# twitter-research/cwn

Hardware: AMD Instinct MI355X
Metric: cells/sec, propagate scope, ZINC-like ring-lifted batch (max_ring 6) (higher is better)
Workload: dtype f32

## Files before the change

cwn_amd/csrc/cwn_layer.hip:

```cpp
#include <hip/hip_runtime.h>
#include <stdint.h>
#include <stddef.h>
#include <mutex>
#include <type_traits>
#include "../../include/cwn_hip.h"
#include "cwn_split.h"

namespace {

using cwn::frag_cd;

#ifdef CWN_LAYER_W8
#undef CWN_LAYER_THREADS
#define CWN_LAYER_THREADS 512
#define CWN_W8 1
#else
#define CWN_W8 0
#endif
#ifndef CWN_LAYER_THREADS
#define CWN_LAYER_THREADS 1024
#endif
#ifndef CWN_LAYER_WEARLY
#define CWN_LAYER_WEARLY -1
#endif
#ifndef CWN_LAYER_NT_STORE
#define CWN_LAYER_NT_STORE 1
#endif
#ifndef CWN_LAYER_WBAR
#define CWN_LAYER_WBAR 1
#endif
constexpr int kThreads = CWN_LAYER_THREADS;
static_assert(kThreads == 512 || kThreads == 1024, "8 or 16 waves");
constexpr int kWaves = kThreads / 64;
constexpr bool kW8 = CWN_W8 != 0;
constexpr int kHS = kThreads == 1024 ? 2 : 1;
constexpr int kWSets = kW8 ? 1 : 2 / kHS;
constexpr size_t kLdsBudget = kW8 ? CWN_LAYER_W8_LDS_BYTES : 160 * 1024;
__host__ __device__ constexpr int gemm_rows_cap(int F) { return kW8 ? CWN_LAYER_W8_GEMM_ROWS(F) : CWN_LAYER_GEMM_ROWS(F); }
__host__ __device__ constexpr int source_rows_cap(int F) { return kW8 ? CWN_LAYER_W8_SOURCE_ROWS(F) : CWN_LAYER_SOURCE_ROWS(F); }
constexpr int kEcap = CWN_LAYER_MAX_ENTRIES;
constexpr int kEI = kEcap / kThreads;
constexpr int kTaskRows = CWN_LAYER_TASK_ROWS;

enum { I_FLAGS = 0, I_G, I_GR0, I_GN, I_CR0, I_CN, I_UE0, I_UNE, I_NT, I_TASK0, I_R1 = 23, I_ROWS, I_B1, I_B2, I_TOTAL };
enum { T_DIM = 0, T_R0, T_N, T_BE0, T_BNE, T_SR0, T_SN, T_INTS };

enum { S_XG = 0, S_XC, S_UP_INDEX, S_UP_SHARED, S_UP_E, S_WP, S_MSG_BIAS, S_PAD, S_TASK0 };
enum { ST_X = 0, ST_XS, ST_OUT_UP, ST_OUT_B, ST_B_INDEX, ST_B_E, ST_EPS1, ST_EPS2, ST_OUT_D, ST_EPS3, ST_FIELDS };
constexpr int kSetFields = S_TASK0 + 2 * ST_FIELDS;
constexpr int kMaxSets = CWN_LAYER_MAX_DIMS;

struct BigSet {
    const int32_t* up_rowptr; const int32_t* up_col; const int32_t* up_aux;
    const int32_t* b_rowptr[2]; const int32_t* b_col[2];
    float* y1; float* y2;
};

struct LayerArgs {
    uint64_t set[kMaxSets][kSetFields];
    const int32_t* items;
    int32_t* err;
    unsigned char* csr_cache;
    int32_t rows_cap;
    int32_t xrows_cap;
    int32_t set_start1, set_start2;
    int32_t lds_limit;
    int32_t store_y;
    BigSet big[kMaxSets];
#ifdef CWN_LAYER_TIMING
    unsigned long long* stamps;
#endif
};

#ifdef CWN_LAYER_TIMING
#define CWN_STAMP_REC 96
#define CWN_STAMP(k)                                                                   \
    do {                                                                               \
        if (threadIdx.x == 0 && A.stamps != nullptr)                                   \
            A.stamps[(size_t)blockIdx.x * CWN_STAMP_REC + (k)] = __builtin_amdgcn_s_memtime();    \
    } while (0)
#define CWN_WSTAMP(k)                                                                  \
    do {                                                                               \
        if ((threadIdx.x & 63) == 0 && A.stamps != nullptr)                            \
            A.stamps[(size_t)blockIdx.x * CWN_STAMP_REC + 16 + 16 * (k) + (threadIdx.x >> 6)] = __builtin_amdgcn_s_memtime(); \
    } while (0)
#define CWN_RSTAMP(k)                                                                  \
    do {                                                                               \
        if ((threadIdx.x & 63) == 0 && A.stamps != nullptr)                            \
            A.stamps[(size_t)blockIdx.x * CWN_STAMP_REC + 64 + 16 * (k) + (threadIdx.x >> 6)] = __builtin_amdgcn_s_memrealtime(); \
    } while (0)
#else
#define CWN_STAMP(k) do { } while (0)
#define CWN_WSTAMP(k) do { } while (0)
#define CWN_RSTAMP(k) do { } while (0)
#endif

template <int F> struct Geo {
    static constexpr int kPlaneStride = F + 8;
    static constexpr int kYStride = F + 4;
    static constexpr int kKS = F / 32;
    static constexpr int kNCT = F / 16;
    static constexpr int kWPC = kWaves / kNCT / kHS;
    static constexpr int kG = F / 4;
    static constexpr int kNG = kThreads / kG;
    static constexpr int kNX = gemm_rows_cap(F) / kNG;
    static constexpr int kNE = source_rows_cap(F) / kNG;
    static_assert(gemm_rows_cap(F) % kNG == 0 && source_rows_cap(F) % kNG == 0, "caps are whole rounds");
    static constexpr int kMaxT = kW8 ? CWN_LAYER_W8_HALF_ROWS(F) / 16 / kWPC : gemm_rows_cap(F) / 16 / kWPC;
    static constexpr int kWChunks = 2 * kKS * 3;
    __host__ __device__ static constexpr size_t planes_bytes(int rows) { return (size_t)3 * rows * kPlaneStride * 2; }
    __host__ __device__ static constexpr size_t xrows_bytes(int rows) { return (size_t)(rows + 1) * F * 4; }
};

constexpr int kRpStride = kTaskRows + 2;
constexpr size_t kCntBytes = ((size_t)3 * kRpStride * 4 + 15) & ~(size_t)15;
constexpr size_t kIdxBytes = kCntBytes + (size_t)3 * kEcap * 2 + (size_t)3 * kRpStride * 2;
constexpr int kCsrSlot = CWN_LAYER_CSR_SLOT_BYTES;
static_assert(kCsrSlot >= 2 * kEcap * 2 + 3 * kRpStride * 2 && kCsrSlot % 16 == 0, "slot holds scol, saux, rowptr");
enum { kSort = 0, kSortStore = 1, kLoad = 2 };

template <int F>
__host__ __device__ constexpr size_t lds_bytes(int rows, int xrows) {
    return Geo<F>::planes_bytes(rows) + Geo<F>::xrows_bytes(xrows) + ((kIdxBytes + 15) & ~(size_t)15);
}

typedef float v4f __attribute__((ext_vector_type(4)));
typedef uint32_t v4u __attribute__((ext_vector_type(4)));
typedef const __attribute__((address_space(1))) float* gcf_p;
typedef __attribute__((address_space(1))) float* gf_p;
typedef const __attribute__((address_space(1))) int64_t* gci64_p;
typedef const __attribute__((address_space(1))) v4f* gcv4_p;
typedef const __attribute__((address_space(1))) v4u* gcu4_p;
typedef __attribute__((address_space(1))) v4f* gv4_p;
typedef const __attribute__((address_space(1))) unsigned char* gcb_p;
typedef __attribute__((address_space(1))) unsigned char* gb_p;
typedef const __attribute__((address_space(1))) uint64_t* gcu64_p;
typedef __attribute__((address_space(1))) v4u* gu4_p;

__device__ __forceinline__ float4 ldg4(gcf_p p) {
    const v4f v = *(gcv4_p)p;
    return make_float4(v.x, v.y, v.z, v.w);
}
__device__ __forceinline__ uint4 ldgu4(gcb_p p) {
    const v4u v = *(gcu4_p)p;
    return make_uint4(v.x, v.y, v.z, v.w);
}
__device__ __forceinline__ void stg4(gf_p p, const float4& a) {
    const v4f v = {a.x, a.y, a.z, a.w};
    *(gv4_p)p = v;
}
__device__ __forceinline__ float4 ldg4o(gcb_p base, uint32_t off) {
    const v4f v = *(gcv4_p)(base + off);
    return make_float4(v.x, v.y, v.z, v.w);
}
__device__ __forceinline__ uint4 ldgu4o(gcb_p base, uint32_t off) {
    const v4u v = *(gcu4_p)(base + off);
    return make_uint4(v.x, v.y, v.z, v.w);
}
__device__ __forceinline__ void stg4o(gb_p base, uint32_t off, const float4& a) {
    const v4f v = {a.x, a.y, a.z, a.w};
#if CWN_LAYER_NT_STORE
    __builtin_nontemporal_store(v, (gv4_p)(base + off));
#else
    *(gv4_p)(base + off) = v;
#endif
}
__device__ __forceinline__ float4 lds4(const float* p) { return *reinterpret_cast<const float4*>(p); }
__device__ __forceinline__ float4 sel4(bool c, const float4& a, const float4& b) {
    return make_float4(c ? a.x : b.x, c ? a.y : b.y, c ? a.z : b.z, c ? a.w : b.w);
}
template <int NX>
__device__ __forceinline__ float4 pick(const float4 (&xv)[NX], int k) {
    float4 r = xv[0];
#pragma unroll
    for (int i = 1; i < NX; ++i) r = sel4(k == i, xv[i], r);
    return r;
}

template <int NR>
struct RowSet { int s[NR], e[NR]; bool on[NR]; };

template <int NR, int NG>
// ... 256 lines not shown
                    for (int i = 0; i < kPer; ++i) {
                        const int lr = gq + i * G::kNG;
                        uint2 ph, pm, pl;
                        cwn::split4(cur[i], ph, pm, pl);
                        uint16_t* dst = bplanes + (size_t)lr * G::kPlaneStride + f;
                        *reinterpret_cast<uint2*>(dst) = ph;
                        *reinterpret_cast<uint2*>(dst + bplane) = pm;
                        *reinterpret_cast<uint2*>(dst + 2 * bplane) = pl;
                    }
                    if (c0 + kCH < n_max) request(nxt, c0 + kCH);
                    __syncthreads();
#pragma unroll
                    for (int hh = 0; hh < kWSets; ++hh) {
                        const int h = kHS == 2 ? my_h : hh;
                        const int rows_h = h == 0 ? g_n : c_n;
                        float* const yb = h == 0 ? Bg.y1 + (size_t)t_r0[0] * F : Bg.y2 + (size_t)c_r0 * F;
                        for (int tl = rt_par; tl < kCH / 16; tl += G::kWPC) {
                            if (c0 + tl * 16 >= rows_h) break;
                            const uint16_t* p0 = bplanes + (size_t)(h * kCH + tl * 16 + l15) * G::kPlaneStride + kq * 8;
                            frag_cd c = {0.f, 0.f, 0.f, 0.f};
#pragma unroll
                            for (int ks = 0; ks < G::kKS; ++ks) {
                                const uint4 xh = *reinterpret_cast<const uint4*>(p0 + ks * 32);
                                const uint4 xm = *reinterpret_cast<const uint4*>(p0 + bplane + ks * 32);
                                const uint4 xl = *reinterpret_cast<const uint4*>(p0 + 2 * bplane + ks * 32);
                                c = cwn::mfma_split6(wsp[hh][ks][0], wsp[hh][ks][1], wsp[hh][ks][2], xh, xm, xl, c);
                            }
                            if (h == 0) { c[0] += bb.x; c[1] += bb.y; c[2] += bb.z; c[3] += bb.w; }
                            const int row = c0 + tl * 16 + l15;
                            if (row < rows_h)
                                *reinterpret_cast<float4*>(yb + (size_t)row * F + ct * 16 + kq * 4) = make_float4(c[0], c[1], c[2], c[3]);
                        }
                    }
#pragma unroll
                    for (int i = 0; i < kPer; ++i) cur[i] = nxt[i];
                }
            }
            __builtin_amdgcn_fence(__ATOMIC_RELEASE, "workgroup");
            __syncthreads();
            __builtin_amdgcn_fence(__ATOMIC_ACQUIRE, "workgroup");
            int32_t* const lidx = reinterpret_cast<int32_t*>(smem);
            const int lcap = A.lds_limit / 4;
            int lused = 0;
            struct Seg { const int32_t* rp; const int32_t* cl; const int32_t* ax; int off; };
            auto stage = [&](const int32_t* rp_g, const int32_t* cl_g, const int32_t* ax_g, int first, int n_rows) {
                if (rp_g == nullptr || n_rows <= 0) return Seg{nullptr, nullptr, nullptr, 0};
                Seg sg{rp_g + first, cl_g, ax_g, 0};
                const int s0 = rp_g[first], e0 = rp_g[first + n_rows], ne = e0 - s0;
                const int need = (n_rows + 1) + ne * (ax_g != nullptr ? 2 : 1);
#ifdef CWN_BIG_NO_STAGE
                if (true) return sg;
#endif
                if (ne < 0 || lused + need > lcap) return sg;
                int32_t* lrp = lidx + lused;
                int32_t* lcl = lrp + n_rows + 1;
                int32_t* lax = lcl + ne;
                for (int i = tid; i <= n_rows; i += kThreads) lrp[i] = rp_g[first + i];
                for (int i = tid; i < ne; i += kThreads) {
                    lcl[i] = cl_g[s0 + i];
                    if (ax_g != nullptr) lax[i] = ax_g[s0 + i];
                }
                lused += need;
                return Seg{lrp, lcl, ax_g != nullptr ? lax : nullptr, s0};
            };
            const Seg su = (has_gemm) ? stage(Bg.up_rowptr, Bg.up_col, Bg.up_aux, t_r0[0], g_n) : Seg{nullptr, nullptr, nullptr, 0};
            Seg sb[2];
#pragma unroll
            for (int t = 0; t < 2; ++t)
                sb[t] = t_bne[t] > 0 ? stage(Bg.b_rowptr[t], Bg.b_col[t], nullptr, t_r0[t], t_n[t]) : Seg{nullptr, nullptr, nullptr, 0};
            __syncthreads();
            bool bad_big = false;
#pragma unroll
            for (int t = 0; t < 2; ++t) {
                if (t_n[t] == 0) continue;
                const gcf_p e1p = (gcf_p)sfld(S_TASK0 + t * ST_FIELDS + ST_EPS1), e2p = (gcf_p)sfld(S_TASK0 + t * ST_FIELDS + ST_EPS2);
                const float eps1 = e1p != (gcf_p)0 ? *e1p : 0.f, eps2 = e2p != (gcf_p)0 ? *e2p : 0.f;
                const gcf_p e3p = (gcf_p)sfld(S_TASK0 + t * ST_FIELDS + ST_EPS3);
                const float eps3 = e3p != (gcf_p)0 ? *e3p : 0.f;
                const gb_p o_d = (gb_p)sfld(S_TASK0 + t * ST_FIELDS + ST_OUT_D);
                const gcb_p xt = (gcb_p)sfld(S_TASK0 + t * ST_FIELDS + ST_X), xs = (gcb_p)sfld(S_TASK0 + t * ST_FIELDS + ST_XS);
                const gb_p o_up = (gb_p)sfld(S_TASK0 + t * ST_FIELDS + ST_OUT_UP), o_b = (gb_p)sfld(S_TASK0 + t * ST_FIELDS + ST_OUT_B);
                const Seg B_ = sb[t];
                const bool upper = t == 0 && has_gemm && su.rp != nullptr;
                const int s_lo = fld(I_TASK0 + t * T_INTS + T_SR0), s_n = t_sn[t];
                for (int r = gq; r < t_n[t]; r += G::kNG) {
                    const int64_t row = (int64_t)t_r0[t] + r;
                    const float4 xi = ldg4o(xt, (uint32_t)row * kRowB + fB);
                    float4 ab = make_float4(0.f, 0.f, 0.f, 0.f);
                    if (B_.rp != nullptr) {
                        const int s_ = B_.rp[r], e_ = B_.rp[r + 1];
                        for (int p = s_; p < e_; p += 4) {
                            int v[4];
                            float4 a[4];
#pragma unroll
                            for (int u = 0; u < 4; ++u) {
                                v[u] = B_.cl[min(p + u, e_ - 1) - B_.off];
                                if ((unsigned)(v[u] - s_lo) >= (unsigned)s_n) { bad_big = true; v[u] = s_lo; }
                            }
#pragma unroll
                            for (int u = 0; u < 4; ++u) a[u] = ldg4o(xs, (uint32_t)v[u] * kRowB + fB);
#pragma unroll
                            for (int u = 0; u < 4; ++u)
                                if (p + u < e_) { ab.x += a[u].x; ab.y += a[u].y; ab.z += a[u].z; ab.w += a[u].w; }
                        }
                    }
                    stg4o(o_b, (uint32_t)row * kRowB + fB, axpy4(ab, 1.0f + eps2, xi));
                    if (o_d != (gb_p)0)
                        stg4o(o_d, (uint32_t)row * kRowB + fB, axpy4(make_float4(0.f, 0.f, 0.f, 0.f), 1.0f + eps3, xi));
                    float4 au = make_float4(0.f, 0.f, 0.f, 0.f);
                    if (upper) {
                        const int s_ = su.rp[r], e_ = su.rp[r + 1];
                        for (int p = s_; p < e_; p += 4) {
                            int j[4], ci[4];
                            float4 y[4], z[4];
#pragma unroll
                            for (int u = 0; u < 4; ++u) {
                                j[u] = su.cl[min(p + u, e_ - 1) - su.off];
                                ci[u] = su.ax[min(p + u, e_ - 1) - su.off];
                                if ((unsigned)(j[u] - t_r0[0]) >= (unsigned)g_n || (unsigned)(ci[u] - c_r0) >= (unsigned)c_n) {
                                    bad_big = true;
                                    j[u] = t_r0[0]; ci[u] = c_r0;
                                }
                            }
#pragma unroll
                            for (int u = 0; u < 4; ++u) {
                                y[u] = *reinterpret_cast<const float4*>(Bg.y1 + (size_t)j[u] * F + f);
                                z[u] = *reinterpret_cast<const float4*>(Bg.y2 + (size_t)ci[u] * F + f);
                            }
#pragma unroll
                            for (int u = 0; u < 4; ++u)
                                if (p + u < e_) {
                                    au.x += fmaxf(y[u].x + z[u].x, 0.0f); au.y += fmaxf(y[u].y + z[u].y, 0.0f);
                                    au.z += fmaxf(y[u].z + z[u].z, 0.0f); au.w += fmaxf(y[u].w + z[u].w, 0.0f);
                                }
                        }
                    }
                    stg4o(o_up, (uint32_t)row * kRowB + fB, axpy4(au, 1.0f + eps1, xi));
                }
            }
            if (bad_big) atomicOr(A.err, CWN_ERR_BIT_BLOCK);
            CWN_RSTAMP(1);
            return;
        }
    }
    const bool fits = kW8 ? ((unsigned)rows_pad <= (unsigned)gemm_rows_cap(F) && (unsigned)x_rows <= (unsigned)source_rows_cap(F) &&
                             lds_bytes<F>(rows_pad, x_rows) <= (size_t)A.lds_limit)
                          : ((unsigned)rows_pad <= (unsigned)rows_cap && (unsigned)x_rows <= (unsigned)xrows_cap);
    if (!fits || (unsigned)total > (unsigned)kEcap ||
        (unsigned)t_n[0] > (unsigned)kTaskRows || (unsigned)t_n[1] > (unsigned)kTaskRows || (unsigned)R1 > (unsigned)rows_pad) {
        if (tid == 0) atomicOr(A.err, CWN_ERR_BIT_BLOCK);
        return;
    }
    bool bad = false;
    if constexpr (MODE != kLoad) {
        for (int i = tid; i < 3 * kRpStride; i += kThreads) ecnt[i] = 0u;
    }

    const gcf_p dummy = (gcf_p)A.items;
    int64_t ek[kEI], ev[kEI], ea[kEI];
    int s1 = 0, s2 = 0, s3 = 0;
    if constexpr (MODE != kLoad) {
        const int u_e0 = fld(I_UE0), t_be0[2] = {fld(I_TASK0 + T_BE0), fld(I_TASK0 + T_INTS + T_BE0)};
        s1 = fld(I_UNE), s2 = b1 + t_bne[0], s3 = b2 + t_bne[1];
        const gci64_p up_index = (gci64_p)sfld(S_UP_INDEX), up_shared = (gci64_p)sfld(S_UP_SHARED);
        const gci64_p b_index0 = (gci64_p)sfld(S_TASK0 + ST_B_INDEX);
        const gci64_p b_index1 = (gci64_p)sfld(S_TASK0 + ST_FIELDS + ST_B_INDEX);
        const int64_t up_E = (int64_t)sfld(S_UP_E);
        const int64_t b_E0 = (int64_t)sfld(S_TASK0 + ST_B_E), b_E1 = (int64_t)sfld(S_TASK0 + ST_FIELDS + ST_B_E);
#pragma unroll
        for (int i = 0; i < kEI; ++i) {
            const int w = tid + i * kThreads;
            const bool in_up = w < s1, in_b0 = w >= b1 && w < s2, in_b1 = w >= b2 && w < s3;
            const gci64_p src = in_up ? up_index : in_b0 ? b_index0 : in_b1 ? b_index1 : (gci64_p)A.items;
            const int64_t E = in_up ? up_E : in_b0 ? b_E0 : in_b1 ? b_E1 : 0;
            const int64_t e = in_up ? (int64_t)u_e0 + w : in_b0 ? (int64_t)t_be0[0] + (w - b1)
                                                       : in_b1 ? (int64_t)t_be0[1] + (w - b2) : 0;
            ev[i] = src[e];
            ek[i] = src[E + e];
            ea[i] = (in_up ? up_shared : (gci64_p)A.items)[in_up ? e : 0];
        }
    }
    uint4 csr_img = make_uint4(0u, 0u, 0u, 0u);
    if constexpr (MODE == kLoad)
        csr_img = ldgu4((gcb_p)A.csr_cache + (size_t)blockIdx.x * kCsrSlot + (size_t)min(tid, kCsrSlot / 16 - 1) * 16);
    float epsv;
    {
        static_assert(ST_EPS2 == ST_EPS1 + 1, "eps1, eps2 are consecutive fields");
        const int k = lane < 4 ? S_TASK0 + ((lane & 2) ? ST_FIELDS : 0) + ST_EPS1 + (lane & 1)
                               : S_TASK0 + ((lane & 1) ? ST_FIELDS : 0) + ST_EPS3;
        const uint64_t bits = (uint64_t)(uint32_t)__builtin_amdgcn_ds_bpermute(4 * k, srec_lo) |
                              ((uint64_t)(uint32_t)__builtin_amdgcn_ds_bpermute(4 * k, srec_hi) << 32);
        const gcf_p ep = lane < 6 ? (gcf_p)bits : (gcf_p)0;
        const float v = *(ep != (gcf_p)0 ? ep : dummy);
        epsv = ep != (gcf_p)0 ? v : 0.0f;
    }
    const gcf_p bias = (gcf_p)sfld(S_MSG_BIAS);
    const bool has_bias = has_gemm && bias != (gcf_p)0;
    CWN_STAMP(11);
    constexpr int kNX = G::kNX, kNE = G::kNE;
    float4 xv[kNX], ev4[kNE];
    {
        const gcb_p xg = (gcb_p)sfld(S_XG) + (size_t)t_r0[0] * kRowB, xc = (gcb_p)sfld(S_XC) + (size_t)fld(I_CR0) * kRowB;
        const gcb_p xs = (gcb_p)sfld(S_TASK0 + ST_XS) + (size_t)fld(I_TASK0 + T_SR0) * kRowB;
        const int nxr = (rows_pad + G::kNG - 1) / G::kNG, ner = (t_sn[0] + G::kNG - 1) / G::kNG;
        const int wave_row0 = wave_u * (64 / G::kG);
        const uint64_t xg_b = (uint64_t)(uintptr_t)xg, xc_b = (uint64_t)(uintptr_t)xc;
#pragma unroll
        for (int i = 0; i < kNX; ++i) {
            if (i < nxr) {
                const bool second = c_n > 0 && i * G::kNG + (G::kNG > 16 ? wave_row0 : 0) >= R1;
                const gcb_p base = (gcb_p)(second ? xc_b : xg_b);
                const int last = (second ? c_n : g_n) - 1, first = second ? i * G::kNG - R1 : i * G::kNG;
                xv[i] = ldg4o(base, (uint32_t)max(min(gq + first, last), 0) * kRowB + fB);
            }
        }
#pragma unroll
        for (int i = 0; i < kNE; ++i) {
            if (i < ner) ev4[i] = ldg4o(xs, (uint32_t)min(gq + i * G::kNG, t_sn[0] - 1) * kRowB + fB);
        }
    }
    CWN_STAMP(12);
    CWN_WSTAMP(1);
    if constexpr (MODE != kLoad) {
        asm volatile("s_waitcnt lgkmcnt(0)" ::: "memory");
        __builtin_amdgcn_s_barrier();
    } else if (CWN_LAYER_WBAR) {
        __builtin_amdgcn_s_barrier();
    }
#pragma unroll
    for (int hh = 0; hh < kWSets; ++hh) {
        const int h = kHS == 2 ? my_h : hh;
#pragma unroll
        for (int ks = kWEarly; ks < G::kKS; ++ks)
#pragma unroll
            for (int pl = 0; pl < 3; ++pl) wsp[hh][ks][pl] = wload(h, ks, pl);
    }
    CWN_STAMP(1);

    unsigned char* const csr_lds = reinterpret_cast<unsigned char*>(scol);
    if constexpr (MODE == kLoad) {
        if (tid < kCsrSlot / 16) *reinterpret_cast<uint4*>(csr_lds + (size_t)tid * 16) = csr_img;
        CWN_STAMP(2);
        CWN_STAMP(3);
    } else {
        const int g_r0 = t_r0[0], c_r0 = fld(I_CR0);
        const int t_sr0[2] = {fld(I_TASK0 + T_SR0), fld(I_TASK0 + T_INTS + T_SR0)};
        int e_seg[kEI], e_row[kEI], e_val[kEI], e_aux[kEI], e_pos[kEI];
    #pragma unroll
        for (int i = 0; i < kEI; ++i) {
            const int w = tid + i * kThreads;
            e_seg[i] = -1;
            e_row[i] = e_val[i] = e_aux[i] = e_pos[i] = 0;
            if (w < total) {
                int64_t k = 0, v = 0, a = 0, nk = 1, nv = 1, na = 1;
                int seg = -1;
                if (w < s1) {
                    seg = 0;
                    k = ek[i] - g_r0; v = ev[i] - g_r0; a = ea[i] - c_r0;
                    nk = g_n; nv = g_n; na = c_n;
                } else if (w >= b1 && w < s2) {
                    seg = 1;
                    k = ek[i] - t_r0[0]; v = ev[i] - t_sr0[0];
                    nk = t_n[0]; nv = t_sn[0];
                } else if (w >= b2 && w < s3) {
                    seg = 2;
                    k = ek[i] - t_r0[1]; v = ev[i] - t_sr0[1];
                    nk = t_n[1];
                    v = (v >= 0 && v < t_sn[1]) ? v + t_sn[0] : -1;
                    nv = t_sn[0] + t_sn[1];
                }
                if (seg >= 0 && (k < 0 || k >= nk || v < 0 || v >= nv || a < 0 || a >= na)) {
                    bad = true;
                    k = 0; v = 0; a = 0;
                }
                if (seg >= 0) {
                    e_seg[i] = seg; e_row[i] = (int)k; e_val[i] = (int)v; e_aux[i] = (int)a;
                    e_pos[i] = (int)atomicAdd(&ecnt[seg * kRpStride + (int)k], 1u);
                }
            }
        }
        if (bad) atomicOr(A.err, CWN_ERR_BIT_BLOCK);
        __syncthreads();
        CWN_STAMP(2);

        if (wave < 3) {
            static_assert(kRpStride <= 4 * 64, "four rows per lane");
            const int n_rows = wave == 0 ? g_n : t_n[wave - 1];
            const uint32_t* c = ecnt + wave * kRpStride;
            uint16_t* rp = rowptr + wave * kRpStride;
            int cj[4], sum = 0;
    #pragma unroll
            for (int j = 0; j < 4; ++j) {
                const int r = 4 * lane + j;
                cj[j] = r < n_rows ? (int)c[r] : 0;
                sum += cj[j];
            }
            int incl = sum;
    #pragma unroll
            for (int off = 1; off < 64; off <<= 1) {
                const int t = __shfl_up(incl, off, 64);
                if (lane >= off) incl += t;
            }
            int run = incl - sum;
    #pragma unroll
            for (int j = 0; j < 4; ++j) {
                const int r = 4 * lane + j;
                if (r <= n_rows) rp[r] = (uint16_t)run;
                run += cj[j];
            }
        }
        __syncthreads();

    #pragma unroll
        for (int i = 0; i < kEI; ++i) {
            if (e_seg[i] >= 0) {
                const int seg0 = e_seg[i] == 0 ? 0 : (e_seg[i] == 1 ? b1 : b2);
                eslot[seg0 + rowptr[e_seg[i] * kRpStride + e_row[i]] + e_pos[i]] = (uint16_t)(tid + i * kThreads);
            }
        }
        __syncthreads();
    #pragma unroll
        for (int i = 0; i < kEI; ++i) {
            if (e_seg[i] >= 0) {
                const int w = tid + i * kThreads;
                const int seg0 = e_seg[i] == 0 ? 0 : (e_seg[i] == 1 ? b1 : b2);
                const uint16_t* rp = rowptr + e_seg[i] * kRpStride + e_row[i];
                const int lo = seg0 + rp[0], hi = seg0 + rp[1];
                int less = 0;
                for (int p = lo; p < hi; ++p) less += (int)eslot[p] < w ? 1 : 0;
                scol[lo + less] = (uint16_t)e_val[i];
                saux[lo + less] = (uint16_t)e_aux[i];
            }
        }
        CWN_STAMP(3);
    }

    {
        const size_t plane = (size_t)rows_cap * G::kPlaneStride;
        const bool copy_src = !kW8 && t_sn[1] > 0;
#pragma unroll
        for (int i = 0; i < kNX; ++i) {
            const int row = gq + i * G::kNG;
            if (has_gemm && (row < g_n || (row >= R1 && row < R1 + c_n))) {
                uint2 ph, pm, pl;
                cwn::split4(xv[i], ph, pm, pl);
                uint16_t* dst = planes + (size_t)row * G::kPlaneStride + f;
                *reinterpret_cast<uint2*>(dst) = ph;
                *reinterpret_cast<uint2*>(dst + plane) = pm;
                *reinterpret_cast<uint2*>(dst + 2 * plane) = pl;
            }
            if (copy_src && row < g_n) *reinterpret_cast<float4*>(xsrc + (size_t)(t_sn[0] + row) * F + f) = xv[i];
        }
#pragma unroll
        for (int i = 0; i < kNE; ++i) {
            const int row = gq + i * G::kNG;
            if (row < t_sn[0]) *reinterpret_cast<float4*>(xsrc + (size_t)row * F + f) = ev4[i];
        }
        if (gq == 0) *reinterpret_cast<float4*>(xsrc + (size_t)x_rows * F + f) = make_float4(0.f, 0.f, 0.f, 0.f);
    }
    CWN_WSTAMP(2);
    __syncthreads();
    if constexpr (MODE == kSortStore) {
        if (tid < kCsrSlot / 16) {
            const uint4 v = *reinterpret_cast<const uint4*>(csr_lds + (size_t)tid * 16);
            const v4u vv = {v.x, v.y, v.z, v.w};
#if CWN_LAYER_NT_STORE
            __builtin_nontemporal_store(vv, (gu4_p)((gb_p)A.csr_cache + (size_t)blockIdx.x * kCsrSlot + (size_t)tid * 16));
#else
            *(gu4_p)((gb_p)A.csr_cache + (size_t)blockIdx.x * kCsrSlot + (size_t)tid * 16) = vv;
#endif
        }
    }
    CWN_STAMP(4);

    float eps1[2], eps2[2];
    eps1[0] = __builtin_bit_cast(float, __builtin_amdgcn_readlane(__builtin_bit_cast(int, epsv), 0));
    eps2[0] = __builtin_bit_cast(float, __builtin_amdgcn_readlane(__builtin_bit_cast(int, epsv), 1));
    eps1[1] = __builtin_bit_cast(float, __builtin_amdgcn_readlane(__builtin_bit_cast(int, epsv), 2));
    eps2[1] = __builtin_bit_cast(float, __builtin_amdgcn_readlane(__builtin_bit_cast(int, epsv), 3));
    const float eps3[2] = {__builtin_bit_cast(float, __builtin_amdgcn_readlane(__builtin_bit_cast(int, epsv), 4)),
                           __builtin_bit_cast(float, __builtin_amdgcn_readlane(__builtin_bit_cast(int, epsv), 5))};
#ifndef CWN_LAYER_NR
#define CWN_LAYER_NR (CWN_LAYER_THREADS == 1024 ? 1 : 2)
#endif
    constexpr int kNR = CWN_LAYER_NR;
    {
        gb_p out_up[2], out_b[2], out_d[2];
        bool has_d[2];
#pragma unroll
        for (int t = 0; t < 2; ++t) {
            out_up[t] = (gb_p)sfld(S_TASK0 + t * ST_FIELDS + ST_OUT_UP) + (size_t)t_r0[t] * kRowB;
            out_b[t] = (gb_p)sfld(S_TASK0 + t * ST_FIELDS + ST_OUT_B) + (size_t)t_r0[t] * kRowB;
            const uint64_t od = sfld(S_TASK0 + t * ST_FIELDS + ST_OUT_D);
            has_d[t] = od != 0;
            out_d[t] = (gb_p)od + (size_t)t_r0[t] * kRowB;
        }
        const uint16_t* const cols[2] = {scol + b1, scol + b2};
        const int sh = G::kNG > 16 ? R1 % G::kNG : 0, k0 = R1 / G::kNG;
        const int gq1 = gq >= sh ? gq - sh : gq - sh + G::kNG, carry1 = gq >= sh ? 0 : 1;
        const bool any_b = t_bne[0] + t_bne[1] > 0;
        const int rounds = (max(t_n[0], t_n[1]) + G::kNG - 1) / G::kNG;
        for (int k = 0; k < rounds; ++k) {
            const int r = gq + k * G::kNG;
            const int rt_[2] = {r, gq1 + k * G::kNG};
            RowSet<2> R;
            int steps = 0;
#pragma unroll
            for (int t = 0; t < 2; ++t) {
                R.on[t] = rt_[t] < t_n[t];
                R.s[t] = R.e[t] = 0;
                if (any_b) {
                    const uint16_t* rp = rowptr + (t + 1) * kRpStride;
                    const int rr = R.on[t] ? rt_[t] : 0;
                    const int s_ = rp[rr], e_ = rp[rr + 1];
                    R.s[t] = R.on[t] ? s_ : 0;
                    R.e[t] = R.on[t] ? e_ : 0;
                    steps = max(steps, R.e[t] - R.s[t]);
                }
            }
            float4 acc[2];
            const float4 xi[2] = {pick(xv, k), pick(xv, k0 + k + carry1)};
            if constexpr (kW8)
                gather_sum_planes<F>(acc, R, steps, cols, xsrc, x_rows, planes, (size_t)rows_cap * G::kPlaneStride, t_sn[0], f);
            else
                gather_sum<2, F>(acc, R, steps, cols, xsrc, x_rows, f);
#pragma unroll
            for (int t = 0; t < 2; ++t) {
                const uint32_t off = (uint32_t)rt_[t] * kRowB + fB;
                if (R.on[t]) {
                    stg4o(out_b[t], off, axpy4(acc[t], 1.0f + eps2[t], xi[t]));
                    if (!(has_gemm && t == 0))
                        stg4o(out_up[t], off, axpy4(make_float4(0.f, 0.f, 0.f, 0.f), 1.0f + eps1[t], xi[t]));
                    if (!kW8 && has_d[t])
                        stg4o(out_d[t], off, axpy4(make_float4(0.f, 0.f, 0.f, 0.f), 1.0f + eps3[t], xi[t]));
                }
            }
        }
        if constexpr (kW8) {
#pragma unroll
            for (int t = 0; t < 2; ++t) {
                if (!has_d[t]) continue;
                const gcb_p xt = (gcb_p)sfld(S_TASK0 + t * ST_FIELDS + ST_X) + (size_t)t_r0[t] * kRowB;
                for (int r = gq; r < t_n[t]; r += G::kNG) {
                    const float4 v = ldg4o(xt, (uint32_t)r * kRowB + fB);
                    stg4o(out_d[t], (uint32_t)r * kRowB + fB, axpy4(make_float4(0.f, 0.f, 0.f, 0.f), 1.0f + eps3[t], v));
                }
            }
        }
    }
    CWN_STAMP(5);
    if (!has_gemm) { CWN_RSTAMP(1); return; }

    float4 b4 = ldg4(has_bias ? bias + ct * 16 + kq * 4 : dummy);
    if (!has_bias) b4 = make_float4(0.f, 0.f, 0.f, 0.f);
    const int T1 = (g_n + 15) >> 4, T2 = (c_n + 15) >> 4;
    if constexpr (kW8) {
        constexpr int kMaxT = G::kMaxT;
        const size_t plane = (size_t)rows_cap * G::kPlaneStride;
        frag_cd acc[2][kMaxT];
        if ((unsigned)T1 > (unsigned)(kMaxT * G::kWPC) || (unsigned)T2 > (unsigned)(kMaxT * G::kWPC)) {
            if (tid == 0) atomicOr(A.err, CWN_ERR_BIT_BLOCK);
            return;
        }
#pragma unroll
        for (int h = 0; h < 2; ++h) {
            const int rt0 = h == 0 ? 0 : R1 / 16, rt1 = rt0 + (h == 0 ? T1 : T2);
            const int first = rt0 + ((rt_par - rt0) % G::kWPC + G::kWPC) % G::kWPC;
#pragma unroll
            for (int j = 0; j < kMaxT; ++j) acc[h][j] = frag_cd{0.f, 0.f, 0.f, 0.f};
#pragma unroll
            for (int ks = 0; ks < G::kKS; ++ks) {
#pragma unroll
                for (int j = 0; j < kMaxT; ++j) {
                    const int rt = first + j * G::kWPC;
                    if (rt < rt1) {
                        const uint16_t* p0 = planes + (size_t)(rt * 16 + l15) * G::kPlaneStride + kq * 8 + ks * 32;
                        const uint4 xh0 = *reinterpret_cast<const uint4*>(p0);
                        const uint4 xm0 = *reinterpret_cast<const uint4*>(p0 + plane);
                        const uint4 xl0 = *reinterpret_cast<const uint4*>(p0 + 2 * plane);
                        acc[h][j] = cwn::mfma_split6(wsp[0][ks][0], wsp[0][ks][1], wsp[0][ks][2], xh0, xm0, xl0, acc[h][j]);
                    }
                }
                if (h == 0) {
#pragma unroll
                    for (int pl = 0; pl < 3; ++pl) wsp[0][ks][pl] = wload(1, ks, pl);
// ... 507 lines not shown
```

Measured before the change: 731.8 million.

## Build per-segment CSR inside three dedicated waves instead of block-wide sorts

When every segment fits in 128 entries, the last three waves each load, count, scan and scatter one segment's CSR entries on their own, using only wave-local LDS waits. This drops the block-wide barriers the rest of the block used to wait on while building CSR. The entry metadata is also packed into two ints. The wide path keeps the old block-wide scheme, and correctness now depends on the packed key limits and on wave-local ordering of LDS accesses.

```diff
diff --git a/cwn_amd/csrc/cwn_layer.hip b/cwn_amd/csrc/cwn_layer.hip
--- a/cwn_amd/csrc/cwn_layer.hip
+++ b/cwn_amd/csrc/cwn_layer.hip
@@ -28,6 +28,9 @@
 #endif
 #ifndef CWN_LAYER_WBAR
 #define CWN_LAYER_WBAR 1
+#endif
+#ifndef CWN_LAYER_SORT_CHUNKS
+#define CWN_LAYER_SORT_CHUNKS 2
 #endif
 constexpr int kThreads = CWN_LAYER_THREADS;
 static_assert(kThreads == 512 || kThreads == 1024, "8 or 16 waves");
@@ -590,13 +593,26 @@
         return;
     }
     bool bad = false;
+    constexpr int kSortChunks = CWN_LAYER_SORT_CHUNKS, kSortLanes = 64 * kSortChunks;
+    constexpr int kES = kEI > kSortChunks ? kEI : kSortChunks;
+    bool wide = false, sorts = false;
+    int my_seg = -1;
     if constexpr (MODE != kLoad) {
-        for (int i = tid; i < 3 * kRpStride; i += kThreads) ecnt[i] = 0u;
-    }
+        wide = max(fld(I_UNE), max(t_bne[0], t_bne[1])) > kSortLanes;
+        my_seg = wave_u - (kWaves - 3);
+        sorts = wide || my_seg >= 0;
+        if (wide) {
+            for (int i = tid; i < 3 * kRpStride; i += kThreads) ecnt[i] = 0u;
+        } else if (sorts) {
+            for (int i = lane; i < kRpStride; i += 64) ecnt[my_seg * kRpStride + i] = 0u;
+        }
+    }
+    const int seg0_my = my_seg <= 0 ? 0 : (my_seg == 1 ? b1 : b2);
+    auto entry_no = [&](int i) { return wide ? (i < kEI ? tid + i * kThreads : kEcap) : seg0_my + i * 64 + lane; };
 
     const gcf_p dummy = (gcf_p)A.items;
-    int64_t ek[kEI], ev[kEI], ea[kEI];
-    int s1 = 0, s2 = 0, s3 = 0;
+    int64_t ek[kES], ev[kES], ea[kES];
+    int s1 = 0, s2 = 0, s3 = 0, n_my = 0;
     if constexpr (MODE != kLoad) {
         const int u_e0 = fld(I_UE0), t_be0[2] = {fld(I_TASK0 + T_BE0), fld(I_TASK0 + T_INTS + T_BE0)};
         s1 = fld(I_UNE), s2 = b1 + t_bne[0], s3 = b2 + t_bne[1];
@@ -605,17 +621,35 @@
         const gci64_p b_index1 = (gci64_p)sfld(S_TASK0 + ST_FIELDS + ST_B_INDEX);
         const int64_t up_E = (int64_t)sfld(S_UP_E);
         const int64_t b_E0 = (int64_t)sfld(S_TASK0 + ST_B_E), b_E1 = (int64_t)sfld(S_TASK0 + ST_FIELDS + ST_B_E);
-#pragma unroll
-        for (int i = 0; i < kEI; ++i) {
-            const int w = tid + i * kThreads;
-            const bool in_up = w < s1, in_b0 = w >= b1 && w < s2, in_b1 = w >= b2 && w < s3;
-            const gci64_p src = in_up ? up_index : in_b0 ? b_index0 : in_b1 ? b_index1 : (gci64_p)A.items;
-            const int64_t E = in_up ? up_E : in_b0 ? b_E0 : in_b1 ? b_E1 : 0;
-            const int64_t e = in_up ? (int64_t)u_e0 + w : in_b0 ? (int64_t)t_be0[0] + (w - b1)
-                                                       : in_b1 ? (int64_t)t_be0[1] + (w - b2) : 0;
-            ev[i] = src[e];
-            ek[i] = src[E + e];
-            ea[i] = (in_up ? up_shared : (gci64_p)A.items)[in_up ? e : 0];
+        if (wide) {
+#pragma unroll
+            for (int i = 0; i < kEI; ++i) {
+                const int w = tid + i * kThreads;
+                const bool in_up = w < s1, in_b0 = w >= b1 && w < s2, in_b1 = w >= b2 && w < s3;
+                const gci64_p src = in_up ? up_index : in_b0 ? b_index0 : in_b1 ? b_index1 : (gci64_p)A.items;
+                const int64_t E = in_up ? up_E : in_b0 ? b_E0 : in_b1 ? b_E1 : 0;
+                const int64_t e = in_up ? (int64_t)u_e0 + w : in_b0 ? (int64_t)t_be0[0] + (w - b1)
+                                                           : in_b1 ? (int64_t)t_be0[1] + (w - b2) : 0;
+                ev[i] = src[e];
+                ek[i] = src[E + e];
+                ea[i] = (in_up ? up_shared : (gci64_p)A.items)[in_up ? e : 0];
+            }
+        } else if (sorts) {
+            const gci64_p src = my_seg == 0 ? up_index : my_seg == 1 ? b_index0 : b_index1;
+            const int64_t E = my_seg == 0 ? up_E : my_seg == 1 ? b_E0 : b_E1;
+            const int64_t e0 = my_seg == 0 ? u_e0 : t_be0[my_seg == 1 ? 0 : 1];
+            n_my = my_seg == 0 ? s1 : my_seg == 1 ? t_bne[0] : t_bne[1];
+            const gcb_p bv = (gcb_p)(n_my > 0 ? src + e0 : (gci64_p)A.items);
+            const gcb_p bk = (gcb_p)(n_my > 0 ? src + E + e0 : (gci64_p)A.items);
+            const gcb_p ba = (gcb_p)(n_my > 0 && my_seg == 0 ? up_shared + e0 : (gci64_p)A.items);
+#pragma unroll
+            for (int i = 0; i < kSortChunks; ++i) {
+                const int j = i * 64 + lane;
+                const uint32_t off = j < n_my ? (uint32_t)j * 8u : 0u;
+                ev[i] = *(gci64_p)(bv + off);
+                ek[i] = *(gci64_p)(bk + off);
+                ea[i] = *(gci64_p)(ba + (my_seg == 0 ? off : 0u));
+            }
         }
     }
     uint4 csr_img = make_uint4(0u, 0u, 0u, 0u);
@@ -659,7 +693,7 @@
     }
     CWN_STAMP(12);
     CWN_WSTAMP(1);
-    if constexpr (MODE != kLoad) {
+    if (MODE != kLoad && wide) {
         asm volatile("s_waitcnt lgkmcnt(0)" ::: "memory");
         __builtin_amdgcn_s_barrier();
     } else if (CWN_LAYER_WBAR) {
@@ -681,94 +715,128 @@
         CWN_STAMP(2);
         CWN_STAMP(3);
     } else {
-        const int g_r0 = t_r0[0], c_r0 = fld(I_CR0);
-        const int t_sr0[2] = {fld(I_TASK0 + T_SR0), fld(I_TASK0 + T_INTS + T_SR0)};
-        int e_seg[kEI], e_row[kEI], e_val[kEI], e_aux[kEI], e_pos[kEI];
+        auto sort_sync = [&]() {
+            if (wide) __syncthreads();
+            else asm volatile("s_waitcnt lgkmcnt(0)" ::: "memory");
+        };
+        const int scan_seg = wide ? wave_u : my_seg;
+        if (sorts) {
+            const int g_r0 = t_r0[0], c_r0 = fld(I_CR0);
+            const int t_sr0[2] = {fld(I_TASK0 + T_SR0), fld(I_TASK0 + T_INTS + T_SR0)};
+            int e_key[kES], e_va[kES];
     #pragma unroll
-        for (int i = 0; i < kEI; ++i) {
-            const int w = tid + i * kThreads;
-            e_seg[i] = -1;
-            e_row[i] = e_val[i] = e_aux[i] = e_pos[i] = 0;
-            if (w < total) {
-                int64_t k = 0, v = 0, a = 0, nk = 1, nv = 1, na = 1;
-                int seg = -1;
-                if (w < s1) {
-                    seg = 0;
-                    k = ek[i] - g_r0; v = ev[i] - g_r0; a = ea[i] - c_r0;
-                    nk = g_n; nv = g_n; na = c_n;
-                } else if (w >= b1 && w < s2) {
-                    seg = 1;
-                    k = ek[i] - t_r0[0]; v = ev[i] - t_sr0[0];
-                    nk = t_n[0]; nv = t_sn[0];
-                } else if (w >= b2 && w < s3) {
-                    seg = 2;
-                    k = ek[i] - t_r0[1]; v = ev[i] - t_sr0[1];
-                    nk = t_n[1];
-                    v = (v >= 0 && v < t_sn[1]) ? v + t_sn[0] : -1;
-                    nv = t_sn[0] + t_sn[1];
-                }
-                if (seg >= 0 && (k < 0 || k >= nk || v < 0 || v >= nv || a < 0 || a >= na)) {
-                    bad = true;
-                    k = 0; v = 0; a = 0;
-                }
-                if (seg >= 0) {
-                    e_seg[i] = seg; e_row[i] = (int)k; e_val[i] = (int)v; e_aux[i] = (int)a;
-                    e_pos[i] = (int)atomicAdd(&ecnt[seg * kRpStride + (int)k], 1u);
-                }
-            }
-        }
-        if (bad) atomicOr(A.err, CWN_ERR_BIT_BLOCK);
-        __syncthreads();
-        CWN_STAMP(2);
-
-        if (wave < 3) {
-            static_assert(kRpStride <= 4 * 64, "four rows per lane");
-            const int n_rows = wave == 0 ? g_n : t_n[wave - 1];
-            const uint32_t* c = ecnt + wave * kRpStride;
-            uint16_t* rp = rowptr + wave * kRpStride;
-            int cj[4], sum = 0;
+            for (int i = 0; i < kES; ++i) {
+                e_key[i] = -1;
+                e_va[i] = 0;
+            }
+            if (wide) {
     #pragma unroll
-            for (int j = 0; j < 4; ++j) {
-                const int r = 4 * lane + j;
-                cj[j] = r < n_rows ? (int)c[r] : 0;
-                sum += cj[j];
-            }
-            int incl = sum;
+                for (int i = 0; i < kEI; ++i) {
+                    const int w = tid + i * kThreads;
+                    if (w < total) {
+                        int64_t k = 0, v = 0, a = 0, nk = 1, nv = 1, na = 1;
+                        int seg = -1;
+                        if (w < s1) {
+                            seg = 0;
+                            k = ek[i] - g_r0; v = ev[i] - g_r0; a = ea[i] - c_r0;
+                            nk = g_n; nv = g_n; na = c_n;
+                        } else if (w >= b1 && w < s2) {
+                            seg = 1;
+                            k = ek[i] - t_r0[0]; v = ev[i] - t_sr0[0];
+                            nk = t_n[0]; nv = t_sn[0];
+                        } else if (w >= b2 && w < s3) {
+                            seg = 2;
+                            k = ek[i] - t_r0[1]; v = ev[i] - t_sr0[1];
+                            nk = t_n[1];
+                            v = (v >= 0 && v < t_sn[1]) ? v + t_sn[0] : -1;
+                            nv = t_sn[0] + t_sn[1];
+                        }
+                        if (seg >= 0 && (k < 0 || k >= nk || v < 0 || v >= nv || a < 0 || a >= na)) {
+                            bad = true;
+                            k = 0; v = 0; a = 0;
+                        }
+                        if (seg >= 0) {
+                            e_va[i] = (int)v | ((int)a << 16);
+                            e_key[i] = (int)k | ((int)atomicAdd(&ecnt[seg * kRpStride + (int)k], 1u) << 8) | (seg << 20);
+                        }
+                    }
+                }
+            } else {
+                const int tt = my_seg == 2 ? 1 : 0;
+                const int64_t k0 = t_r0[tt], v0 = my_seg == 0 ? g_r0 : t_sr0[tt];
+                const uint64_t nk = (uint64_t)t_n[tt], nv0 = (uint64_t)(my_seg == 0 ? g_n : t_sn[tt]);
+                const uint64_t na = (uint64_t)(my_seg == 0 ? c_n : 1);
+                const int vsh = my_seg == 2 ? t_sn[0] : 0;
+                asm volatile("s_waitcnt lgkmcnt(0)" ::: "memory");
     #pragma unroll
-            for (int off = 1; off < 64; off <<= 1) {
-                const int t = __shfl_up(incl, off, 64);
-                if (lane >= off) incl += t;
-            }
-            int run = incl - sum;
+                for (int i = 0; i < kSortChunks; ++i) {
+                    if (i * 64 + lane < n_my) {
+                        const uint64_t k = (uint64_t)(ek[i] - k0), v = (uint64_t)(ev[i] - v0), a = my_seg == 0 ? (uint64_t)(ea[i] - c_r0) : 0;
+                        const bool ok = k < nk && v < nv0 && a < na;
+                        bad = bad || !ok;
+                        const int kr = ok ? (int)k : 0;
+                        e_va[i] = ok ? ((int)v + vsh) | ((int)a << 16) : 0;
+                        e_key[i] = kr | ((int)atomicAdd(&ecnt[my_seg * kRpStride + kr], 1u) << 8) | (my_seg << 20);
+                    }
+                }
+            }
+            if (bad) atomicOr(A.err, CWN_ERR_BIT_BLOCK);
+            sort_sync();
+            CWN_STAMP(2);
+
+            if ((unsigned)scan_seg < 3u) {
+                static_assert(kRpStride <= 4 * 64 && kTaskRows < 256 && kEcap <= 4096, "four rows per lane; the packed entry key");
+                const int n_rows = scan_seg == 0 ? g_n : t_n[scan_seg - 1];
+                const uint32_t* c = ecnt + scan_seg * kRpStride;
+                uint16_t* rp = rowptr + scan_seg * kRpStride;
+                int cj[4], sum = 0;
     #pragma unroll
-            for (int j = 0; j < 4; ++j) {
-                const int r = 4 * lane + j;
-                if (r <= n_rows) rp[r] = (uint16_t)run;
-                run += cj[j];
-            }
-        }
-        __syncthreads();
-
+                for (int j = 0; j < 4; ++j) {
+                    const int r = 4 * lane + j;
+                    cj[j] = r < n_rows ? (int)c[r] : 0;
+                    sum += cj[j];
+                }
+                int incl = sum;
     #pragma unroll
-        for (int i = 0; i < kEI; ++i) {
-            if (e_seg[i] >= 0) {
-                const int seg0 = e_seg[i] == 0 ? 0 : (e_seg[i] == 1 ? b1 : b2);
-                eslot[seg0 + rowptr[e_seg[i] * kRpStride + e_row[i]] + e_pos[i]] = (uint16_t)(tid + i * kThreads);
-            }
-        }
-        __syncthreads();
+                for (int off = 1; off < 64; off <<= 1) {
+                    const int t = __shfl_up(incl, off, 64);
+                    if (lane >= off) incl += t;
+                }
+                int run = incl - sum;
     #pragma unroll
-        for (int i = 0; i < kEI; ++i) {
-            if (e_seg[i] >= 0) {
-                const int w = tid + i * kThreads;
-                const int seg0 = e_seg[i] == 0 ? 0 : (e_seg[i] == 1 ? b1 : b2);
-                const uint16_t* rp = rowptr + e_seg[i] * kRpStride + e_row[i];
-                const int lo = seg0 + rp[0], hi = seg0 + rp[1];
-                int less = 0;
-                for (int p = lo; p < hi; ++p) less += (int)eslot[p] < w ? 1 : 0;
-                scol[lo + less] = (uint16_t)e_val[i];
-                saux[lo + less] = (uint16_t)e_aux[i];
-            }
+                for (int j = 0; j < 4; ++j) {
+                    const int r = 4 * lane + j;
+                    if (r <= n_rows) rp[r] = (uint16_t)run;
+                    run += cj[j];
+                }
+            }
+            sort_sync();
+
+    #pragma unroll
+            for (int i = 0; i < kES; ++i) {
+                if (e_key[i] >= 0) {
+                    const int seg = e_key[i] >> 20, row = e_key[i] & 255, pos = (e_key[i] >> 8) & 4095;
+                    const int seg0 = seg == 0 ? 0 : (seg == 1 ? b1 : b2);
+                    eslot[seg0 + rowptr[seg * kRpStride + row] + pos] = (uint16_t)entry_no(i);
+                }
+            }
+            sort_sync();
+    #pragma unroll
+            for (int i = 0; i < kES; ++i) {
+                if (e_key[i] >= 0) {
+                    const int w = entry_no(i);
+                    const int seg = e_key[i] >> 20, row = e_key[i] & 255;
+                    const int seg0 = seg == 0 ? 0 : (seg == 1 ? b1 : b2);
+                    const uint16_t* rp = rowptr + seg * kRpStride + row;
+                    const int lo = seg0 + rp[0], hi = seg0 + rp[1];
+                    int less = 0;
+                    for (int p = lo; p < hi; ++p) less += (int)eslot[p] < w ? 1 : 0;
+                    scol[lo + less] = (uint16_t)e_va[i];
+                    saux[lo + less] = (uint16_t)((unsigned)e_va[i] >> 16);
+                }
+            }
+        } else {
+            CWN_STAMP(2);
         }
         CWN_STAMP(3);
     }
```

Result: slower. 721.1 million (-1.5%).
